# sipposip/pr-disagg-radar-gan

Hardware: AMD Instinct MI355X
Metric: cWGAN-GP train samples/sec, 24x16x16 tiles, bs=256 (higher is better)
Workload: dtype f32; 1 GPU; ndomain=16, 24h, bs=256 fp32, 1 critic step + 1 gen step (BASELINE configs[1]); batch_per_gpu=256, global_batch=256, n_critic=1, parallelism=dp1, world=1, rccl_ranks_seen=1, weights=random init (RandomNormal 0.02 / glorot_uniform), dropout 0.25 active

## Files before the change

pr_disagg_radar_gan_amd/csrc/rdgan_api.hip:

```cpp
#include <hip/hip_runtime.h>
#include <stdio.h>
#include <string.h>
#include <math.h>
#include <string>
#include <vector>
#include <algorithm>
#include <unordered_set>

#include "../../include/rdgan.h"
#include "rdgan_plan.h"
#include "rdgan_hostplan.h"
#include "rdgan_rng.h"
#include "rdgan_gemm.hip.h"
#include "rdgan_gemm_ws.hip.h"
#include "rdgan_gemm_ws16.hip.h"
#include "rdgan_gemm_f16.hip.h"
#include "rdgan_upconv16.hip.h"
#include "rdgan_upconv16b.hip.h"
#include "rdgan_upconv16t.hip.h"
#include "rdgan_elem.hip.h"
#include "rdgan_data.hip.h"
#include "rdgan_edge.hip.h"
#include "rdgan_d2slab16.hip.h"
#include "rdgan_d2fwd16.hip.h"
// ... 79 lines not shown
  float* dw6_part;
  int side_on = 1;
  int split3 = 0;
  int dense_slices = 0;
  uint64_t gver_in = 0, cver_in = 0;
  const float* gcache_ptr = nullptr; uint64_t gcache_ver = 0; int gcache_cfg = -1;
  const float* ccache_ptr = nullptr; uint64_t ccache_ver = 0; int ccache_cfg = -1;
  long form_builds[2] = {0, 0};
  int keep_gates = 0;
  void* gate_keep[5] = {nullptr, nullptr, nullptr, nullptr, nullptr};
  int gate_keep_B = 0;
  hipStream_t side = nullptr;
  hipEvent_t ev_fork = nullptr, ev_join = nullptr, ev_cw = nullptr, ev_g[4] = {nullptr, nullptr, nullptr, nullptr};
  int* d_flag;
  int fwd_ahead = -1;
  hipStream_t ahead = nullptr;
  hipEvent_t ev_ahead_fork = nullptr, ev_ahead_done = nullptr;
  float* kpartial_ahead = nullptr;
  int* flag_ahead = nullptr;
  bool ahead_pending = false;
  const float *ahead_gp = nullptr, *ahead_z = nullptr, *ahead_cond = nullptr;
  int ahead_B = 0;
  uint64_t ahead_gver = 0;
  std::unordered_set<const void*> lds_attr_done;
  int prof_launches = 0;
  std::vector<RdLaunchRec> launch_recs;
  size_t launch_used = 0;
  char cur_kernel[48] = {0};
  double flops_acc = 0;
  unsigned prof_mask = 0;
  std::vector<hipEvent_t> ev_start[RDGAN_NUM_TAGS], ev_stop[RDGAN_NUM_TAGS];
  size_t ev_used[RDGAN_NUM_TAGS] = {0};
};

#define RD_CHECK(h, call)                                                        \
  do {                                                                           \
    hipError_t e_ = (call);                                                      \
    if (e_ != hipSuccess) {                                                      \
      char b_[512];                                                              \
      snprintf(b_, sizeof b_, "%s:%d %s -> %s", __FILE__, __LINE__, #call, hipGetErrorString(e_)); \
      if (h) (h)->err = b_;                                                      \
      return (int)e_;                                                            \
    }                                                                            \
  } while (0)
#define RD_TRY(expr)            \
  do {                          \
// ... 689 lines not shown
    h->DWT[0] = h->DWT[1] = nullptr;
    for (int l = 2; l <= 4; ++l) carve(h->DWT[l], 27L * dch[l - 1] * dch[l]);
    carve(h->W1T, 64 * h->ldp1);
    carve(h->W1P, 27L * h->CP * 64); carve(h->dW1P, 27L * h->CP * 64);
    h->GWT[0] = nullptr;
    for (int l = 1; l <= 3; ++l) carve(h->GWT[l], 27L * gch[l - 1] * gch[l]);
    carve(h->W9T, 64 * 32);
    h->GWC[0] = h->GWD[0] = nullptr;
    for (int l = 1; l <= 3; ++l) { carve(h->GWC[l], 64L * gch[l - 1] * gch[l]); carve(h->GWD[l], 64L * gch[l - 1] * gch[l]); }
    carve(h->dWc, 64L * 256 * 256);
    {
      size_t ne = 0, ns = 0;
      for (int l = 1; l <= 3; ++l) {
        const int* sd = h->gdim[l - 1];
        ne = std::max(ne, (size_t)(sd[0] + 1) * sd[1] * sd[2] * gch[l - 1]);
        ns = std::max(ns, (size_t)sd[0] * 4 * sd[1] * sd[2] * gch[l]);
      }
      h->fE[0] = h->fU[0] = nullptr;
      for (int l = 1; l <= 3; ++l) {
        const int* sd = h->gdim[l - 1];
        carve(h->fE[l], MB * (size_t)(sd[0] + 1) * sd[1] * sd[2] * gch[l - 1]);
        carve(h->fU[l], 48L * gch[l - 1] * gch[l]);
      }
      carve(h->fdE, MB * ne); carve(h->fgS, MB * ns);
      {
        float* p = nullptr;
        h->bU[0] = nullptr;
        for (int l = 1; l <= 3; ++l) { carve(p, 24L * gch[l - 1] * gch[l] + 8); h->bU[l] = p; }
        carve(p, 24L * 256 * 256 + 8); h->bUT = p;
        const long KP128 = (h->n_in + 127) / 128 * 128;
        carve(p, (long)((MB + 31) / 32 * 32) * KP128 / 2 + 8); h->xcat16 = p;
        carve(p, (long)h->n_nodes * KP128 / 2 + 8); h->bW0 = p;
        h->bWF[0] = h->bWF[1] = h->bWB[0] = h->bWB[1] = nullptr;
        for (int l = 2; l <= 4; ++l) {
          carve(p, 27L * dch[l - 1] * dch[l] / 2 + 8); h->bWF[l] = p;
          carve(p, 27L * dch[l - 1] * dch[l] / 2 + 8); h->bWB[l] = p;
        }
        h->bG1F[0] = nullptr;
        for (int l = 1; l <= 3; ++l) { carve(p, 32L * gch[l - 1] * gch[l] + 8); h->bG1F[l] = p; }
        carve(p, 32L * 256 * 256 + 8); h->bG1B = p;
        h->fWF[0] = h->fWF[1] = h->fWB[0] = h->fWB[1] = h->fG1F[0] = nullptr;
        for (int l = 2; l <= 4; ++l) {
          carve(p, 27L * dch[l - 1] * dch[l] / 2 + 8); h->fWF[l] = p;
          carve(p, 27L * dch[l - 1] * dch[l] / 2 + 8); h->fWB[l] = p;
        }
        for (int l = 1; l <= 3; ++l) { carve(p, 32L * gch[l - 1] * gch[l] + 8); h->fG1F[l] = p; }
        carve(p, 32L * 256 * 256 + 8); h->fG1B = p;
// ... 8 lines not shown
      }
      carve(h->fdU, 48L * 256 * 256); carve(h->fUT, 48L * 256 * 256);
    }
    { float* f = nullptr; carve(f, 64); if (pass == 1) { h->d_flag = (int*)f; h->flag_ahead = (int*)f + 32; } }
    carve(h->g9b_tmp, 64);
    carve(h->ubias_part, 32 * 8 * 64);
    carve(h->gp_part, (size_t)MB * 64);
    carve(h->dw6_part, (size_t)16 * h->F);
    if (pass == 0) {
      h->ws_bytes = off + 256;
      e = hipMalloc((void**)&h->ws, h->ws_bytes);
      if (e != hipSuccess) { (void)hipFree(h->d_plans); delete h; return (int)e; }
      (void)hipMemset(h->ws, 0, h->ws_bytes);
    }
  }
  {
    bool ok = hipStreamCreateWithFlags(&h->side, hipStreamNonBlocking) == hipSuccess;
    hipEvent_t* evs[] = {&h->ev_fork, &h->ev_join, &h->ev_cw, &h->ev_g[1], &h->ev_g[2], &h->ev_g[3]};
    for (hipEvent_t* e2 : evs) ok = ok && hipEventCreateWithFlags(e2, hipEventDisableTiming) == hipSuccess;
    if (!ok) { h->side_on = 0; (void)hipGetLastError(); }
    bool ok2 = hipStreamCreateWithFlags(&h->ahead, hipStreamNonBlocking) == hipSuccess;
    ok2 = ok2 && hipEventCreateWithFlags(&h->ev_ahead_fork, hipEventDisableTiming) == hipSuccess;
    ok2 = ok2 && hipEventCreateWithFlags(&h->ev_ahead_done, hipEventDisableTiming) == hipSuccess;
    if (!ok2) { h->ahead = nullptr; (void)hipGetLastError(); }
  }
  *out = h;
  return 0;
}

extern "C" void rdgan_destroy(rdgan_handle* h) {
  if (!h) return;
  if (h->side) { (void)hipStreamSynchronize(h->side); (void)hipStreamDestroy(h->side); }
  if (h->ahead) { (void)hipStreamSynchronize(h->ahead); (void)hipStreamDestroy(h->ahead); }
  for (hipEvent_t e2 : {h->ev_fork, h->ev_join, h->ev_cw, h->ev_g[1], h->ev_g[2], h->ev_g[3], h->ev_ahead_fork, h->ev_ahead_done})
    if (e2) (void)hipEventDestroy(e2);
  for (auto& r : h->launch_recs) { (void)hipEventDestroy(r.e0); (void)hipEventDestroy(r.e1); }
  for (int t = 0; t < RDGAN_NUM_TAGS; ++t) {
    for (auto e : h->ev_start[t]) (void)hipEventDestroy(e);
    for (auto e : h->ev_stop[t]) (void)hipEventDestroy(e);
  }
  for (void* g : h->gate_keep) if (g) (void)hipFree(g);
  if (h->ws) (void)hipFree(h->ws);
  if (h->d_plans) (void)hipFree(h->d_plans);
  if (h->d_tab) (void)hipFree(h->d_tab);
  delete h;
}

extern "C" const char* rdgan_last_error(const rdgan_handle* h) { return h ? h->err.c_str() : "null handle"; }
extern "C" long rdgan_gen_param_count(const rdgan_handle* h) { return h ? h->n_gen : -1; }
extern "C" long rdgan_critic_param_count(const rdgan_handle* h) { return h ? h->n_critic : -1; }
extern "C" long rdgan_workspace_bytes(const rdgan_handle* h) { return h ? (long)h->ws_bytes : -1; }
extern "C" int rdgan_gen_param_layout(const rdgan_handle* h, long* offsets, long* sizes) {
  if (!h) return -2;
  for (int i = 0; i < 10; ++i) { if (offsets) offsets[i] = h->goff[i]; if (sizes) sizes[i] = h->gsz[i]; }
  return 10;
}
extern "C" int rdgan_critic_param_layout(const rdgan_handle* h, long* offsets, long* sizes) {
// ... 26 lines not shown
  if (!strcmp(name, "d2_wgrad_slab")) { h->d2_wgrad_slab = value ? 1 : 0; return 0; }
  if (!strcmp(name, "upwgrad_slab")) { h->upwgrad_slab = value ? 1 : 0; return 0; }
  if (!strcmp(name, "d1_dgrad_fused")) { h->d1_dgrad_fused = value ? 1 : 0; return 0; }
  if (!strcmp(name, "d1_wgrad16")) { h->d1_wgrad16 = value ? 1 : 0; return 0; }
  if (!strcmp(name, "wgrad_wide")) { h->wgrad_wide = value ? 1 : 0; return 0; }
  if (!strcmp(name, "conv_f16")) {
    if (value < 0 || value > 2) return bad_arg(h, "conv_f16: 0, 1 or 2 (2: regardless of the launch size)");
    h->conv_f16 = value; h->ccache_ver = 0; h->gcache_ver = 0; return 0;
  }
  if (!strcmp(name, "d2_fwd_slab")) { h->d2_fwd_slab = value ? 1 : 0; h->ccache_ver = 0; return 0; }
  if (!strcmp(name, "d2_gate_bits")) { h->d2_gate_bits = value ? 1 : 0; return 0; }
  if (!strcmp(name, "d2_slab")) { h->d2_slab = value ? 1 : 0; h->ccache_ver = 0; return 0; }
  if (!strcmp(name, "dense_wgrad_slices")) { h->dense_slices = value; return 0; }
  if (!strcmp(name, "keep_gates")) {
    h->keep_gates = value ? 1 : 0;
    h->gate_keep_B = 0;
    for (int l = 1; l <= 4 && h->keep_gates; ++l)
      if (!h->gate_keep[l]) RD_CHECK(h, hipMalloc(&h->gate_keep[l], (size_t)h->MB * h->dL[l] * h->dch[l] * sizeof(float)));
    return 0;
  }
  if (!strcmp(name, "split3")) { h->split3 = value ? 1 : 0; return 0; }
  if (!strcmp(name, "side_stream")) { h->side_on = (value && h->side) ? 1 : 0; return 0; }
  if (!strcmp(name, "gen_fwd_ahead")) { h->fwd_ahead = value < 0 ? -1 : (value ? 1 : 0); return 0; }
  if (!strcmp(name, "edge_kernels")) { h->edge_kernels = value < 0 ? 0 : (value > 2 ? 2 : value); return 0; }
  if (!strcmp(name, "sample_offset")) { if (value < 0) return bad_arg(h, "set_option: sample_offset < 0"); h->sample_offset = value; return 0; }
  if (!strcmp(name, "ws_ksplit")) { h->ws_ksplit = value < 0 ? 0 : (value > 8 ? 8 : value); return 0; }
  return bad_arg(h, "set_option: unknown option");
}

extern "C" int rdgan_set_weight_versions(rdgan_handle* h, uint64_t gen_version, uint64_t critic_version) {
  if (!h) return -2;
  h->gver_in = gen_version; h->cver_in = critic_version;
  return 0;
}
extern "C" int rdgan_form_builds(const rdgan_handle* h, long* gen_builds, long* critic_builds) {
  if (!h) return -2;
  if (gen_builds) *gen_builds = h->form_builds[0];
  if (critic_builds) *critic_builds = h->form_builds[1];
  return 0;
}

extern "C" int rdgan_profile(rdgan_handle* h, unsigned tag_mask) {
  if (!h) return -2;
  h->prof_mask = tag_mask;
  for (int t = 0; t < RDGAN_NUM_TAGS; ++t) {
    h->ev_used[t] = 0;
// ... 433 lines not shown
    e.gw = nd; e.ghw = nd * nd; e.gq = gq;
    if (a16) RD_TRY(launch_conv_a16(h, h->plans[PL_G9F], h->d_plans + PL_G9F, B, h->h3, h->W9T, 32, h->P9, e, st, -1, true, false));
    else
    RD_TRY(launch_conv(h, h->plans[PL_G9F], h->d_plans + PL_G9F, B, h->h3, h->W9T, 32, h->P9, e, st, -1));
    ProfScope ps(h, RDGAN_TAG_ELEMENTWISE, st);
    if (gq == 3) hipLaunchKernelGGL((k_tapsum_softmax<RDGAN_NHOURS, 3>), dim3((unsigned)((ncol + 63) / 64)), dim3(256), 0, st, h->P9,
                                    gp + h->goff[9], out, B, nd, nd, h->d_flag);
    else hipLaunchKernelGGL((k_tapsum_softmax<RDGAN_NHOURS, 9>), dim3((unsigned)((ncol + 63) / 64)), dim3(256), 0, st, h->P9,
                            gp + h->goff[9], out, B, nd, nd, h->d_flag);
  } else {
    if (a16) RD_TRY(launch_conv_a16(h, h->plans[PL_G9F], h->d_plans + PL_G9F, B, h->h3, h->W9T, 32, h->P9, epi_make(RD_EPI_PLAIN), st, -1,
                                    true, false));
    else
    RD_TRY(launch_conv(h, h->plans[PL_G9F], h->d_plans + PL_G9F, B, h->h3, h->W9T, 32, h->P9, epi_make(RD_EPI_PLAIN), st, -1));
    ProfScope ps(h, RDGAN_TAG_ELEMENTWISE, st);
    hipLaunchKernelGGL(k_colgather_softmax, dim3((unsigned)((ncol + 63) / 64)), dim3(64), 0, st, h->P9, gp + h->goff[9],
                       out, B, RDGAN_NHOURS, nd, nd, h->d_flag);
  }
  RD_CHECK(h, hipGetLastError());
  return 0;
}

static bool fwd_ahead_on(const rdgan_handle* h) { return h->ahead && h->ev_ahead_done && (h->fwd_ahead < 0 ? !h->a16 : h->fwd_ahead); }

static int ahead_drain(rdgan_handle* h, hipStream_t st) {
  if (!h->ahead_pending) return 0;
  h->ahead_pending = false;
  RD_CHECK(h, hipStreamWaitEvent(st, h->ev_ahead_done, 0));
  return 0;
}

static int ahead_issue(rdgan_handle* h, const float* gp, const float* z, const float* cond, int B, hipStream_t st) {
  RD_CHECK(h, hipEventRecord(h->ev_ahead_fork, st));
  RD_CHECK(h, hipStreamWaitEvent(h->ahead, h->ev_ahead_fork, 0));
  std::swap(h->kpartial, h->kpartial_ahead);
  std::swap(h->d_flag, h->flag_ahead);
  const int rc = gen_forward_impl(h, gp, z, cond, h->fake, B, h->ahead, h->ahead);
  std::swap(h->kpartial, h->kpartial_ahead);
  std::swap(h->d_flag, h->flag_ahead);
  RD_TRY(rc);
  RD_CHECK(h, hipEventRecord(h->ev_ahead_done, h->ahead));
  h->ahead_pending = true;
  h->ahead_gp = gp; h->ahead_z = z; h->ahead_cond = cond; h->ahead_B = B; h->ahead_gver = h->gver_in;
  return 0;
}

// ... 457 lines not shown
  h->ahead_pending = false;
  h->gate_keep_B = 0;
  if (!h->collapse)
    for (int l = 1; l <= 3; ++l)
      RD_TRY(launch_transpose(h, gp + h->goff[2 * l], h->GWT[l], 27, h->gch[l - 1], h->gch[l], h->gch[l - 1], st));
  hipStream_t ws = side_fork(h, st);
  if (!ahead) RD_TRY(gen_forward_impl(h, gp, z, cond, h->fake, B, st, ws));
  if (critic_ready_event) RD_CHECK(h, hipStreamWaitEvent(ws, (hipEvent_t)critic_ready_event, 0));
  RD_TRY(prep_critic_weights(h, dp, ws));
  RD_TRY(side_join(h, st, h->ev_cw));
  if (ahead) {
    RD_CHECK(h, hipStreamWaitEvent(st, h->ev_ahead_done, 0));
    std::swap(h->d_flag, h->flag_ahead);
  }
  {
    ProfScope ps(h, RDGAN_TAG_ELEMENTWISE, st);
    launch_build_critic_input(h, nullptr, h->fake, cond, B, 1, 0u, 0u, st);
  }
  RD_TRY(critic_forward_impl(h, dp, B, seed, st));
  RD_TRY(critic_dgrad_chain(h, dp, B, B, 1, seed, st));
  RD_TRY(critic_input_grad(h, dp, h->du[1], B, st));
  const bool a16 = h->a16 != 0;
  const long npix3 = (long)B * h->gpix[3];
  {
    ProfScope ps(h, RDGAN_TAG_ELEMENTWISE, st);
    long ncol = (long)B * nd * nd;
    hipLaunchKernelGGL(k_softmax_bwd, dim3((unsigned)((ncol + 63) / 64)), dim3(64), 0, st, h->fake, h->g0, h->dl, B,
                       RDGAN_NHOURS, nd, nd);
  }
  const size_t g9_lds = 4 * (size_t)(nd + 2) * (nd + 2) * sizeof(float);
  const bool g9_direct = h->g9_direct && g9_lds <= 96 * 1024 &&
                         (size_t)B * (RDGAN_NHOURS / 2) * 1728 <= h->wpartial_cap;
  if (a16 && !g9_direct) return bad_arg(h, "bf16 storage mode needs the direct backward of the last conv (g9_direct)");
  if (g9_direct) {
    ProfScope ps(h, RDGAN_TAG_GCONV_WGRAD, st);
    const size_t lds = std::max<size_t>(g9_lds, 4 * 27 * 16 * sizeof(f32x4));
    RD_TRY(ensure_lds(h, a16 ? (const void*)k_g9_bwd_pairs<rd_bf16_t> : (const void*)k_g9_bwd_pairs<float>, 96 * 1024));
    int nwg;
    if (h->edge_kernels && g9w_mfma_ok(nd, npix3) && (size_t)std::min<long>((npix3 + 127) / 128, 768) * 1728 <= h->wpartial_cap) {
      const size_t lds_m = g9w_mfma_lds(a16);
      RD_TRY(ensure_lds(h, a16 ? (const void*)k_g9_wgrad_mfma<rd_bf16_t> : (const void*)k_g9_wgrad_mfma<float>, lds_m));
      nwg = (int)std::min<long>((npix3 + 127) / 128, 768);
      LaunchScope ls(h, PL_G9B, RD_KIND_WGRAD, B, 2.0 * npix3 * 64 * 27, st);
      RD_KNAME(h, "k_g9_wgrad_mfma<%s>", a16 ? "bf16" : "f32");
      h->flops_acc += 2.0 * npix3 * 64 * 27;
      if (a16) hipLaunchKernelGGL(k_g9_wgrad_mfma<rd_bf16_t>, dim3(nwg), dim3(256), lds_m, st, h->dl, (const rd_bf16_t*)h->h3, h->wpartial,
                                  npix3, RDGAN_NHOURS, nd, nd, ilog2(nd));
      else hipLaunchKernelGGL(k_g9_wgrad_mfma<float>, dim3(nwg), dim3(256), lds_m, st, h->dl, (const float*)h->h3, h->wpartial,
                              npix3, RDGAN_NHOURS, nd, nd, ilog2(nd));
    } else {
      RD_TRY(ensure_lds(h, a16 ? (const void*)k_g9_wgrad_pairs<rd_bf16_t> : (const void*)k_g9_wgrad_pairs<float>, 96 * 1024));
      const int nunits = B * (RDGAN_NHOURS / 2);
      nwg = std::min(nunits, 3072);
      if (a16) hipLaunchKernelGGL(k_g9_wgrad_pairs<rd_bf16_t>, dim3(nwg), dim3(256), lds, st, h->dl, (const rd_bf16_t*)h->h3, h->wpartial,
                                  RDGAN_NHOURS, nd, nd, nunits);
      else hipLaunchKernelGGL(k_g9_wgrad_pairs<float>, dim3(nwg), dim3(256), lds, st, h->dl, (const float*)h->h3, h->wpartial,
                              RDGAN_NHOURS, nd, nd, nunits);
    }
    hipLaunchKernelGGL(k_reduce_partials, dim3((1728 + 15) / 16), dim3(rd_reduce_threads(nwg)), 0, st, h->wpartial, nwg, 1728, grad + h->goff[8]);
  } else {
    {
      ProfScope ps(h, RDGAN_TAG_ELEMENTWISE, st);
      hipLaunchKernelGGL(k_dl_im2col, dim3(ew_blocks(npix3 * 8)), dim3(256), 0, st, h->dl, h->P9, B, RDGAN_NHOURS, nd, nd);
    }
    RD_TRY(launch_wgrad(h, h->plans[PL_G9B], h->d_plans + PL_G9B, B, h->P9, h->h3, grad + h->goff[8], h->wpartial,
                        h->wpartial_cap, st, RDGAN_TAG_GCONV_WGRAD));
    RD_TRY(launch_conv(h, h->plans[PL_G9B], h->d_plans + PL_G9B, B, h->P9, gp + h->goff[8], 64, h->gh3,
                       epi_make(RD_EPI_PLAIN), st, RDGAN_TAG_GCONV_DGRAD));
  }
  {
    hipStream_t cs = side_fork(h, st);
    RD_TRY(launch_colsum(h, h->dl, npix3 / 64, 64, h->g9b_tmp, cs));
    RD_TRY(launch_colsum(h, h->g9b_tmp, 64, 1, grad + h->goff[9], cs));
  }
  float* hs[4] = {h->h0, h->h1, h->h2, h->h3};
  float* rs[4] = {nullptr, h->r1, h->r2, h->r3};
  float* dys[4] = {nullptr, h->dy1, h->dy2, h->gh3};
  float* gups[4] = {nullptr, h->gup1, h->gup2, h->gup3};
  const int col = h->collapse;
  if (col) {
    RdSliceMap map;
    collapsed_dgrad_slice_map(map.src);
    for (int l = 1; l <= 3; ++l) {
      if (gen_block_fast(h, l, fast_bwd_on(h))) continue;
      if (gen_block_fast(h, l, fast_fwd_on(h)))
        hipLaunchKernelGGL(k_collapse_weights, dim3(ew_blocks(16L * h->gch[l - 1] * h->gch[l])), dim3(256), 0, st,
                           gp + h->goff[2 * l], h->GWC[l], h->gch[l - 1] * h->gch[l]);
      if (a16) continue;
      hipLaunchKernelGGL(k_transpose_map, dim3((h->gch[l] + 31) / 32, (h->gch[l - 1] + 31) / 32, 64), dim3(256), 0, st,
                         h->GWC[l], h->GWD[l], h->gch[l - 1], h->gch[l], map);
    }
  }
  for (int l = 3; l >= 1; --l) {
    const bool fast = gen_block_fast(h, l, fast_bwd_on(h));
    if (l == 3 && g9_direct) {
      ProfScope ps(h, RDGAN_TAG_ELEMENTWISE, st);
      if (a16 && !fast && h->g9_bwd_mfma && (nd * nd) % 32 == 0) {
        const int PP = nd <= 16 ? 4 : 1;
        const size_t lds9 = (size_t)(2 * PP + 2) * (nd + 2) * (nd + 2) * sizeof(float);
        const int nunits = B * (RDGAN_NHOURS / 2 / PP);
        RD_TRY(ensure_lds(h, (const void*)k_g9_bwd_mfma16, lds9));
        hipLaunchKernelGGL(k_g9_bwd_mfma16, dim3((unsigned)std::min(nunits, PP > 1 ? 768 : 1536)), dim3(256), lds9, st, h->dl, gp + h->goff[8],
                           (const rd_bf16_t*)hs[3], rs[3], (rd_bf16_t*)dys[3], nunits, RDGAN_NHOURS, nd, nd, PP);
      } else
      if (a16) hipLaunchKernelGGL(k_g9_bwd_pairs<rd_bf16_t>, dim3(B * (RDGAN_NHOURS / 2)), dim3(256), g9_lds, st, h->dl, gp + h->goff[8],
                                  (const rd_bf16_t*)hs[3], rs[3], (rd_bf16_t*)dys[3], fast ? (rd_bf16_t*)h->fgS : (rd_bf16_t*)nullptr,
                                  RDGAN_NHOURS, nd, nd);
      else hipLaunchKernelGGL(k_g9_bwd_pairs<float>, dim3(B * (RDGAN_NHOURS / 2)), dim3(256), g9_lds, st, h->dl, gp + h->goff[8],
                              (const float*)hs[3], rs[3], dys[3], fast ? h->fgS : (float*)nullptr, RDGAN_NHOURS, nd, nd);
      RD_CHECK(h, hipGetLastError());
    } else if (fast) {
      ProfScope ps(h, RDGAN_TAG_ELEMENTWISE, st);
      const long HW = (long)h->gdim[l][1] * h->gdim[l][2];
      RD_TRY(launch_pn_bwd_pairs(h, l == 3 ? h->gh3 : gups[l + 1], hs[l], rs[l], dys[l], h->fgS, (long)B * h->gdim[l - 1][0] * HW,
                                 HW, h->gch[l], st, a16));
    } else {
      ProfScope ps(h, RDGAN_TAG_ELEMENTWISE, st);
      if (l == 3) RD_TRY(launch_pn_bwd(h, h->gh3, hs[3], rs[3], dys[3], npix3, 64, 0, 0, 0, 0, st, a16));
      else RD_TRY(launch_pn_bwd(h, gups[l + 1], hs[l], rs[l], dys[l], (long)B * h->gpix[l], h->gch[l], col ? 0 : 1,
                                h->gdim[l][0], h->gdim[l][1], h->gdim[l][2], st, a16));
    }
    const long cc = (long)h->gch[l - 1] * h->gch[l];
    if (fast) {
      const int* sd = h->gdim[l - 1];
      const int D = sd[0];
      const long P = (long)sd[1] * sd[2] * h->gch[l - 1];
      RdWeightMap wm;
      fastd_weight_map(wm);
      {
        ProfScope ps(h, RDGAN_TAG_ELEMENTWISE, st);
        if (!gen_block_fast(h, l, fast_fwd_on(h))) {
          const dim3 dg(ew_blocks((long)B * (D + 1) * P / 4));
          if (a16) hipLaunchKernelGGL(k_diff_d<rd_bf16_t>, dg, dim3(256), 0, st, (const rd_bf16_t*)hs[l - 1], (rd_bf16_t*)h->fE[l], B, D, P);
          else
          hipLaunchKernelGGL(k_diff_d<float>, dg, dim3(256), 0, st, (const float*)hs[l - 1],
                             h->fE[l], B, D, P);
          hipLaunchKernelGGL(k_weight_transform, dim3(ew_blocks(48L * cc / 4)), dim3(256), 0, st, gp + h->goff[2 * l], h->fU[l],
                             (int)cc, 48, wm);
        }
      }
      const float* wsrc[3] = {h->fE[l], hs[l - 1], h->fE[l]};
      const float* wdy[3] = {dys[l], h->fgS, dys[l]};
      for (int g = 0; g < 3; ++g) {
        int pl = PL_F1WA + 3 * g + l - 1;
        if (!a16 && h->wgrad_boxes && h->border_boxes && h->wave_spec && wgrad_box_ok(h->plans[PL_F1WAX + 3 * g + l - 1]) &&
            (h->border_boxes >= 2 || plan_flops(h->plans[PL_F1WAX + 3 * g + l - 1], 1) < 0.8 * plan_flops(h->plans[pl], 1)))
          pl = PL_F1WAX + 3 * g + l - 1;
        if (a16) {
          if (!wgrad16_ok(h->plans[pl], B)) return bad_arg(h, "bf16 storage mode: no bf16 weight-gradient tile for this block");
          RD_TRY(launch_wgrad16(h, h->plans[pl], h->d_plans + pl, B, wsrc[g], wdy[g], h->fdU, h->wpartial, h->wpartial_cap, st,
                                RDGAN_TAG_GCONV_WGRAD));
        } else
        RD_TRY(launch_wgrad(h, h->plans[pl], h->d_plans + pl, B, wsrc[g], wdy[g], h->fdU, h->wpartial, h->wpartial_cap, st,
                            RDGAN_TAG_GCONV_WGRAD));
      }
      hipLaunchKernelGGL(k_weight_transform_adj, dim3(ew_blocks(27L * cc / 4)), dim3(256), 0, st, h->fdU, grad + h->goff[2 * l],
                         (int)cc, 48, wm);
      RD_TRY(launch_colsum(h, dys[l], (long)B * h->gpix[l], h->gch[l], grad + h->goff[2 * l + 1], side_fork(h, st), a16));
      const int pbs = PL_F1BS + l - 1, pbe = PL_F1BE + l - 1;
      RdEpi eb = epi_make(RD_EPI_PLAIN);
      eb.out16 = a16;
      if (a16) {
        RdSliceMap map;
        fastd_dgrad_slice_map(map.src);
        {
          ProfScope ps(h, RDGAN_TAG_ELEMENTWISE, st);
          hipLaunchKernelGGL(k_blocks_to_bf16, dim3((unsigned)std::min<long>((cc / 8 + 255) / 256, 64), 48), dim3(256), 0, st,
                             h->fU[l], (unsigned short*)h->bUT, cc, map);
        }
        RD_TRY(launch_conv16(h, h->plans[pbs], h->d_plans + pbs, B, h->fgS, h->bUT, gups[l], eb, st, RDGAN_TAG_GCONV_DGRAD));
        RD_TRY(launch_conv16(h, h->plans[pbe], h->d_plans + pbe, B, dys[l], h->bUT, h->fdE, eb, st, RDGAN_TAG_GCONV_DGRAD));
      } else {
        {
          RdSliceMap map;
          fastd_dgrad_slice_map(map.src);
          hipLaunchKernelGGL(k_transpose_map, dim3((h->gch[l] + 31) / 32, (h->gch[l - 1] + 31) / 32, 48), dim3(256), 0, st, h->fU[l],
                             h->fUT, h->gch[l - 1], h->gch[l], map);
        }
        RD_TRY(launch_conv(h, h->plans[pbs], h->d_plans + pbs, B, h->fgS, h->fUT, h->gch[l - 1], gups[l], eb, st,
                           RDGAN_TAG_GCONV_DGRAD));
        RD_TRY(launch_conv(h, h->plans[pbe], h->d_plans + pbe, B, dys[l], h->fUT, h->gch[l - 1], h->fdE, eb, st,
                           RDGAN_TAG_GCONV_DGRAD));
      }
      {
        ProfScope ps(h, RDGAN_TAG_ELEMENTWISE, st);
        const dim3 cg(ew_blocks((long)B * D * P / 4));
        if (a16) hipLaunchKernelGGL(k_combine_dx<rd_bf16_t>, cg, dim3(256), 0, st, (rd_bf16_t*)gups[l], (const rd_bf16_t*)h->fdE, B, D, P);
        else hipLaunchKernelGGL(k_combine_dx<float>, cg, dim3(256), 0, st, gups[l], (const float*)h->fdE, B, D, P);
      }
    } else if (col) {
      int plf = PL_G1FC + l - 1, plb = gen_box_plan(h, PL_G1BC + l - 1, PL_G1BCX + l - 1, B);
      const int plfx = PL_G1FCX + l - 1;
      const bool wbox = h->wgrad_boxes && h->border_boxes && h->wave_spec && wgrad_box_ok(h->plans[plfx]) &&
                        (h->border_boxes >= 2 || plan_flops(h->plans[plfx], 1) < 0.8 * plan_flops(h->plans[plf], 1));
      bool bias_done = false;
      if (a16 && l == 3 && h->upwgrad_slab && h->nd == 16) {
        ProfScope ps(h, RDGAN_TAG_GCONV_WGRAD, st);
        LaunchScope ls(h, plf, RD_KIND_WGRAD, B, plan_flops(h->plans[plf], B), st);
        RD_KNAME(h, "k_upconv_wgrad_slab16<bf16>");
        h->flops_acc += plan_flops(h->plans[plf], B);
        const int G = 6 * B >= 64 ? 32 : 8;
        if ((size_t)G * 64 * RD_UWG_TILE > h->wpartial_cap) return bad_arg(h, "upconv wgrad: partial workspace too small");
        RD_TRY(ensure_lds(h, (const void*)k_upconv_wgrad_slab16, RD_UWG_LDS));
        hipLaunchKernelGGL(k_upconv_wgrad_slab16, dim3(8 * G), dim3(512), RD_UWG_LDS, st, (const rd_bf16_t*)hs[l - 1],
                           (const rd_bf16_t*)dys[l], h->wpartial, B, G, h->ubias_part);
        hipLaunchKernelGGL(k_upconv_wgrad_fold, dim3(64 * RD_UWG_TILE / 4 / 256), dim3(256), 0, st, h->wpartial, G, h->dWc);
        hipLaunchKernelGGL(k_reduce_partials, dim3(64 / 16), dim3(rd_reduce_threads(8 * G)), 0, st, h->ubias_part, 8 * G, 64, grad + h->goff[2 * l + 1]);
        bias_done = true;
        RD_CHECK(h, hipGetLastError());
      } else if (a16 && l == 2 && h->upwgrad_slab && h->nd == 16) {
        ProfScope ps(h, RDGAN_TAG_GCONV_WGRAD, st);
        LaunchScope ls(h, plf, RD_KIND_WGRAD, B, plan_flops(h->plans[plf], B), st);
        RD_KNAME(h, "k_upconv2_wgrad_slab16<bf16>");
        h->flops_acc += plan_flops(h->plans[plf], B);
        const int G = 8;
        if ((size_t)G * 64 * RD_UW2_TILE > h->wpartial_cap) return bad_arg(h, "upconv wgrad: partial workspace too small");
        RD_TRY(ensure_lds(h, (const void*)k_upconv2_wgrad_slab16, RD_UW2_LDS));
        hipLaunchKernelGGL(k_upconv2_wgrad_slab16, dim3(32 * G), dim3(512), RD_UW2_LDS, st, (const rd_bf16_t*)hs[l - 1],
                           (const rd_bf16_t*)dys[l], h->wpartial, B, G, h->ubias_part);
        hipLaunchKernelGGL(k_upconv2_wgrad_fold, dim3(64 * RD_UW2_TILE / 4 / 256), dim3(256), 0, st, h->wpartial, G, h->dWc);
        hipLaunchKernelGGL(k_reduce_partials, dim3(128 / 16), dim3(rd_reduce_threads(8 * G)), 0, st, h->ubias_part, 8 * G, 128, grad + h->goff[2 * l + 1]);
        bias_done = true;
        RD_CHECK(h, hipGetLastError());
      } else if (a16) {
        if (wbox && wgrad16_ok(h->plans[plfx], B)) plf = plfx;
        if (!wgrad16_ok(h->plans[plf], B)) return bad_arg(h, "bf16 storage mode: no bf16 weight-gradient tile for this block");
        RD_TRY(launch_wgrad16(h, h->plans[plf], h->d_plans + plf, B, hs[l - 1], dys[l], h->dWc, h->wpartial, h->wpartial_cap, st,
                              RDGAN_TAG_GCONV_WGRAD));
      } else {
      if (wbox) plf = plfx;
      RD_TRY(launch_wgrad(h, h->plans[plf], h->d_plans + plf, B, hs[l - 1], dys[l], h->dWc, h->wpartial, h->wpartial_cap,
                          st, RDGAN_TAG_GCONV_WGRAD));
      }
      hipLaunchKernelGGL(k_fold_collapsed_wgrad, dim3(ew_blocks(27L * cc / 4)), dim3(256), 0, st, h->dWc,
                         grad + h->goff[2 * l], (int)cc);
      if (!bias_done)
      RD_TRY(launch_colsum(h, dys[l], (long)B * h->gpix[l], h->gch[l], grad + h->goff[2 * l + 1], side_fork(h, st), a16));
      if (a16) {
        RdSliceMap map;
        collapsed_dgrad_slice_map(map.src);
        hipLaunchKernelGGL(k_blocks_to_bf16, dim3((unsigned)std::min<long>((cc / 8 + 255) / 256, 64), 64), dim3(256), 0, st,
                           h->GWC[l], (unsigned short*)h->bG1B, cc, map, h->conv_f16 ? (unsigned short*)h->fG1B : nullptr, h->gch[l]);
        RdEpi eb = epi_make(RD_EPI_PLAIN);
        eb.out16 = 1;
        RD_TRY(launch_conv16(h, h->plans[plb], h->d_plans + plb, B, dys[l], h->bG1B, gups[l], eb, st, RDGAN_TAG_GCONV_DGRAD,
                             h->conv_f16 ? h->fG1B : nullptr));
      } else
      RD_TRY(launch_conv(h, h->plans[plb], h->d_plans + plb, B, dys[l], h->GWD[l], h->gch[l - 1], gups[l],
                         epi_make(RD_EPI_PLAIN), st, RDGAN_TAG_GCONV_DGRAD));
    } else {
      int plf = PL_G1F + l - 1, plb = PL_G1B + l - 1;
      RD_TRY(launch_wgrad(h, h->plans[plf], h->d_plans + plf, B, hs[l - 1], dys[l], grad + h->goff[2 * l], h->wpartial,
                          h->wpartial_cap, st, RDGAN_TAG_GCONV_WGRAD));
      RD_TRY(launch_colsum(h, dys[l], (long)B * h->gpix[l], h->gch[l], grad + h->goff[2 * l + 1], side_fork(h, st)));
      RD_TRY(launch_conv(h, h->plans[plb], h->d_plans + plb, B, dys[l], h->GWT[l], h->gch[l - 1], gups[l],
                         epi_make(RD_EPI_PLAIN), st, RDGAN_TAG_GCONV_DGRAD));
    }
  }
  {
    ProfScope ps(h, RDGAN_TAG_ELEMENTWISE, st);
    const dim3 lg(ew_blocks((long)B * h->gpix[0] * 64));
    if (col && a16)
      hipLaunchKernelGGL(k_lrelu_bwd<rd_bf16_t>, lg, dim3(256), 0, st, (const rd_bf16_t*)h->gup1, (const rd_bf16_t*)h->h0, h->ga0,
                         (long)B * h->gpix[0] * 64);
    else if (col)
      hipLaunchKernelGGL(k_lrelu_bwd<float>, lg, dim3(256), 0, st, (const float*)h->gup1, (const float*)h->h0, h->ga0,
                         (long)B * h->gpix[0] * 64);
    else
      hipLaunchKernelGGL(k_pool_lrelu_bwd, lg, dim3(256), 0, st, h->gup1, h->h0,
                         h->ga0, (long)B * h->gpix[0], h->gdim[0][0], h->gdim[0][1], h->gdim[0][2], 256);
  }
  RD_TRY(launch_wgrad(h, h->plans[PL_GDENSE], h->d_plans + PL_GDENSE, B, h->xcat, h->ga0, grad + h->goff[0], h->wpartial,
                      h->wpartial_cap, st, RDGAN_TAG_GCONV_WGRAD));
  RD_TRY(launch_colsum(h, h->ga0, B, h->n_nodes, grad + h->goff[1], side_fork(h, st)));
  RD_TRY(side_join(h, st, h->ev_join));
  {
    ProfScope ps(h, RDGAN_TAG_ELEMENTWISE, st);
    hipLaunchKernelGGL(k_gen_loss, dim3(1), dim3(256), 0, st, h->v, grad + h->n_gen, B, h->d_flag);
  }
  RD_CHECK(h, hipGetLastError());
  return 0;
}

extern "C" int rdgan_adam(float* params, const float* grad, float* v, long n, int t, float lr, float beta2, float eps,
                          float grad_scale, void* stream) {
  if (!params || !grad || !v || n < 1 || t < 1) return -2;
  float lr_t = lr * sqrtf(1.0f - powf(beta2, (float)t));
  hipLaunchKernelGGL(k_adam, dim3(ew_blocks(n / 4 + 1)), dim3(256), 0, (hipStream_t)stream, params, grad, v, n, lr_t, beta2,
                     eps, grad_scale);
  return (int)hipGetLastError();
}

struct TmpPlan {
  RdPlan host; RdPlan* dev = nullptr; RdRow* tab = nullptr;
  int upload() {
    std::vector<RdRow> t;
    if (!plan_build_tables(host, t)) return -2;
    hipError_t e = hipMalloc((void**)&tab, sizeof(RdRow) * t.size());
// ... 776 lines not shown
```

Before: 23580 samples/s.

## Fork generator weight-gradient kernels onto a second stream to overlap data-gradient chain

Generator backward weight-gradient launches (last conv, fast-path blocks, upconv blocks, dense layer) move onto the 'ahead' stream, forked by events from the main stream. The data-gradient convs stay on the main stream, so the two chains can run concurrently. A second fgS scratch buffer, used by block 2, plus per-buffer events stop the overlapping blocks from overwriting a shared buffer, and a join event merges the streams before the loss kernel. It is on by default only in fp32 mode (not a16). It costs extra events, workspace and possible contention for compute units between the streams.

```diff
diff --git a/pr_disagg_radar_gan_amd/csrc/rdgan_api.hip b/pr_disagg_radar_gan_amd/csrc/rdgan_api.hip
--- a/pr_disagg_radar_gan_amd/csrc/rdgan_api.hip
+++ b/pr_disagg_radar_gan_amd/csrc/rdgan_api.hip
@@ -125,6 +125,9 @@
   const float *ahead_gp = nullptr, *ahead_z = nullptr, *ahead_cond = nullptr;
   int ahead_B = 0;
   uint64_t ahead_gver = 0;
+  int wgrad_fork = -1;
+  hipEvent_t ev_wg_fork = nullptr, ev_wg_join = nullptr, ev_fgs[2] = {nullptr, nullptr};
+  float* fgS2 = nullptr;
   std::unordered_set<const void*> lds_attr_done;
   int prof_launches = 0;
   std::vector<RdLaunchRec> launch_recs;
@@ -860,7 +863,7 @@
         carve(h->fE[l], MB * (size_t)(sd[0] + 1) * sd[1] * sd[2] * gch[l - 1]);
         carve(h->fU[l], 48L * gch[l - 1] * gch[l]);
       }
-      carve(h->fdE, MB * ne); carve(h->fgS, MB * ns);
+      carve(h->fdE, MB * ne); carve(h->fgS, MB * ns); carve(h->fgS2, MB * ns);
       {
         float* p = nullptr;
         h->bU[0] = nullptr;
@@ -915,6 +918,8 @@
     bool ok2 = hipStreamCreateWithFlags(&h->ahead, hipStreamNonBlocking) == hipSuccess;
     ok2 = ok2 && hipEventCreateWithFlags(&h->ev_ahead_fork, hipEventDisableTiming) == hipSuccess;
     ok2 = ok2 && hipEventCreateWithFlags(&h->ev_ahead_done, hipEventDisableTiming) == hipSuccess;
+    for (hipEvent_t* e2 : {&h->ev_wg_fork, &h->ev_wg_join, &h->ev_fgs[0], &h->ev_fgs[1]})
+      ok2 = ok2 && hipEventCreateWithFlags(e2, hipEventDisableTiming) == hipSuccess;
     if (!ok2) { h->ahead = nullptr; (void)hipGetLastError(); }
   }
   *out = h;
@@ -925,7 +930,8 @@
   if (!h) return;
   if (h->side) { (void)hipStreamSynchronize(h->side); (void)hipStreamDestroy(h->side); }
   if (h->ahead) { (void)hipStreamSynchronize(h->ahead); (void)hipStreamDestroy(h->ahead); }
-  for (hipEvent_t e2 : {h->ev_fork, h->ev_join, h->ev_cw, h->ev_g[1], h->ev_g[2], h->ev_g[3], h->ev_ahead_fork, h->ev_ahead_done})
+  for (hipEvent_t e2 : {h->ev_fork, h->ev_join, h->ev_cw, h->ev_g[1], h->ev_g[2], h->ev_g[3], h->ev_ahead_fork, h->ev_ahead_done,
+                        h->ev_wg_fork, h->ev_wg_join, h->ev_fgs[0], h->ev_fgs[1]})
     if (e2) (void)hipEventDestroy(e2);
   for (auto& r : h->launch_recs) { (void)hipEventDestroy(r.e0); (void)hipEventDestroy(r.e1); }
   for (int t = 0; t < RDGAN_NUM_TAGS; ++t) {
@@ -998,6 +1004,7 @@
   if (!strcmp(name, "split3")) { h->split3 = value ? 1 : 0; return 0; }
   if (!strcmp(name, "side_stream")) { h->side_on = (value && h->side) ? 1 : 0; return 0; }
   if (!strcmp(name, "gen_fwd_ahead")) { h->fwd_ahead = value < 0 ? -1 : (value ? 1 : 0); return 0; }
+  if (!strcmp(name, "gen_wgrad_fork")) { h->wgrad_fork = value < 0 ? -1 : (value ? 1 : 0); return 0; }
   if (!strcmp(name, "edge_kernels")) { h->edge_kernels = value < 0 ? 0 : (value > 2 ? 2 : value); return 0; }
   if (!strcmp(name, "sample_offset")) { if (value < 0) return bad_arg(h, "set_option: sample_offset < 0"); h->sample_offset = value; return 0; }
   if (!strcmp(name, "ws_ksplit")) { h->ws_ksplit = value < 0 ? 0 : (value > 8 ? 8 : value); return 0; }
@@ -1477,6 +1484,9 @@
 }
 
 static bool fwd_ahead_on(const rdgan_handle* h) { return h->ahead && h->ev_ahead_done && (h->fwd_ahead < 0 ? !h->a16 : h->fwd_ahead); }
+static bool wgrad_fork_on(const rdgan_handle* h) {
+  return h->ahead && h->ev_wg_fork && h->ev_wg_join && h->ev_fgs[1] && (h->wgrad_fork < 0 ? !h->a16 : h->wgrad_fork);
+}
 
 static int ahead_drain(rdgan_handle* h, hipStream_t st) {
   if (!h->ahead_pending) return 0;
@@ -1980,6 +1990,15 @@
   RD_TRY(critic_input_grad(h, dp, h->du[1], B, st));
   const bool a16 = h->a16 != 0;
   const long npix3 = (long)B * h->gpix[3];
+  const bool wfork = wgrad_fork_on(h);
+  hipStream_t wb = st;
+  auto wgrad_branch = [&]() -> int {
+    if (!wfork) return 0;
+    RD_CHECK(h, hipEventRecord(h->ev_wg_fork, st));
+    RD_CHECK(h, hipStreamWaitEvent(h->ahead, h->ev_wg_fork, 0));
+    wb = h->ahead;
+    return 0;
+  };
   {
     ProfScope ps(h, RDGAN_TAG_ELEMENTWISE, st);
     long ncol = (long)B * nd * nd;
@@ -1991,7 +2010,8 @@
                          (size_t)B * (RDGAN_NHOURS / 2) * 1728 <= h->wpartial_cap;
   if (a16 && !g9_direct) return bad_arg(h, "bf16 storage mode needs the direct backward of the last conv (g9_direct)");
   if (g9_direct) {
-    ProfScope ps(h, RDGAN_TAG_GCONV_WGRAD, st);
+    RD_TRY(wgrad_branch());
+    ProfScope ps(h, RDGAN_TAG_GCONV_WGRAD, wb);
     const size_t lds = std::max<size_t>(g9_lds, 4 * 27 * 16 * sizeof(f32x4));
     RD_TRY(ensure_lds(h, a16 ? (const void*)k_g9_bwd_pairs<rd_bf16_t> : (const void*)k_g9_bwd_pairs<float>, 96 * 1024));
     int nwg;
@@ -1999,30 +2019,31 @@
       const size_t lds_m = g9w_mfma_lds(a16);
       RD_TRY(ensure_lds(h, a16 ? (const void*)k_g9_wgrad_mfma<rd_bf16_t> : (const void*)k_g9_wgrad_mfma<float>, lds_m));
       nwg = (int)std::min<long>((npix3 + 127) / 128, 768);
-      LaunchScope ls(h, PL_G9B, RD_KIND_WGRAD, B, 2.0 * npix3 * 64 * 27, st);
+      LaunchScope ls(h, PL_G9B, RD_KIND_WGRAD, B, 2.0 * npix3 * 64 * 27, wb);
       RD_KNAME(h, "k_g9_wgrad_mfma<%s>", a16 ? "bf16" : "f32");
       h->flops_acc += 2.0 * npix3 * 64 * 27;
-      if (a16) hipLaunchKernelGGL(k_g9_wgrad_mfma<rd_bf16_t>, dim3(nwg), dim3(256), lds_m, st, h->dl, (const rd_bf16_t*)h->h3, h->wpartial,
+      if (a16) hipLaunchKernelGGL(k_g9_wgrad_mfma<rd_bf16_t>, dim3(nwg), dim3(256), lds_m, wb, h->dl, (const rd_bf16_t*)h->h3, h->wpartial,
                                   npix3, RDGAN_NHOURS, nd, nd, ilog2(nd));
-      else hipLaunchKernelGGL(k_g9_wgrad_mfma<float>, dim3(nwg), dim3(256), lds_m, st, h->dl, (const float*)h->h3, h->wpartial,
+      else hipLaunchKernelGGL(k_g9_wgrad_mfma<float>, dim3(nwg), dim3(256), lds_m, wb, h->dl, (const float*)h->h3, h->wpartial,
                               npix3, RDGAN_NHOURS, nd, nd, ilog2(nd));
     } else {
       RD_TRY(ensure_lds(h, a16 ? (const void*)k_g9_wgrad_pairs<rd_bf16_t> : (const void*)k_g9_wgrad_pairs<float>, 96 * 1024));
       const int nunits = B * (RDGAN_NHOURS / 2);
       nwg = std::min(nunits, 3072);
-      if (a16) hipLaunchKernelGGL(k_g9_wgrad_pairs<rd_bf16_t>, dim3(nwg), dim3(256), lds, st, h->dl, (const rd_bf16_t*)h->h3, h->wpartial,
+      if (a16) hipLaunchKernelGGL(k_g9_wgrad_pairs<rd_bf16_t>, dim3(nwg), dim3(256), lds, wb, h->dl, (const rd_bf16_t*)h->h3, h->wpartial,
                                   RDGAN_NHOURS, nd, nd, nunits);
-      else hipLaunchKernelGGL(k_g9_wgrad_pairs<float>, dim3(nwg), dim3(256), lds, st, h->dl, (const float*)h->h3, h->wpartial,
+      else hipLaunchKernelGGL(k_g9_wgrad_pairs<float>, dim3(nwg), dim3(256), lds, wb, h->dl, (const float*)h->h3, h->wpartial,
                               RDGAN_NHOURS, nd, nd, nunits);
     }
-    hipLaunchKernelGGL(k_reduce_partials, dim3((1728 + 15) / 16), dim3(rd_reduce_threads(nwg)), 0, st, h->wpartial, nwg, 1728, grad + h->goff[8]);
+    hipLaunchKernelGGL(k_reduce_partials, dim3((1728 + 15) / 16), dim3(rd_reduce_threads(nwg)), 0, wb, h->wpartial, nwg, 1728, grad + h->goff[8]);
   } else {
     {
       ProfScope ps(h, RDGAN_TAG_ELEMENTWISE, st);
       hipLaunchKernelGGL(k_dl_im2col, dim3(ew_blocks(npix3 * 8)), dim3(256), 0, st, h->dl, h->P9, B, RDGAN_NHOURS, nd, nd);
     }
+    RD_TRY(wgrad_branch());
     RD_TRY(launch_wgrad(h, h->plans[PL_G9B], h->d_plans + PL_G9B, B, h->P9, h->h3, grad + h->goff[8], h->wpartial,
-                        h->wpartial_cap, st, RDGAN_TAG_GCONV_WGRAD));
+                        h->wpartial_cap, wb, RDGAN_TAG_GCONV_WGRAD));
     RD_TRY(launch_conv(h, h->plans[PL_G9B], h->d_plans + PL_G9B, B, h->P9, gp + h->goff[8], 64, h->gh3,
                        epi_make(RD_EPI_PLAIN), st, RDGAN_TAG_GCONV_DGRAD));
   }
@@ -2049,8 +2070,12 @@
                          h->GWC[l], h->GWD[l], h->gch[l - 1], h->gch[l], map);
     }
   }
+  bool fgs_branch[2] = {false, false};
   for (int l = 3; l >= 1; --l) {
     const bool fast = gen_block_fast(h, l, fast_bwd_on(h));
+    const int fgi = wfork && l == 2 ? 1 : 0;
+    float* const fgs = fgi ? h->fgS2 : h->fgS;
+    if (fast && fgs_branch[fgi]) RD_CHECK(h, hipStreamWaitEvent(st, h->ev_fgs[fgi], 0));
     if (l == 3 && g9_direct) {
       ProfScope ps(h, RDGAN_TAG_ELEMENTWISE, st);
       if (a16 && !fast && h->g9_bwd_mfma && (nd * nd) % 32 == 0) {
@@ -2062,15 +2087,15 @@
                            (const rd_bf16_t*)hs[3], rs[3], (rd_bf16_t*)dys[3], nunits, RDGAN_NHOURS, nd, nd, PP);
       } else
       if (a16) hipLaunchKernelGGL(k_g9_bwd_pairs<rd_bf16_t>, dim3(B * (RDGAN_NHOURS / 2)), dim3(256), g9_lds, st, h->dl, gp + h->goff[8],
-                                  (const rd_bf16_t*)hs[3], rs[3], (rd_bf16_t*)dys[3], fast ? (rd_bf16_t*)h->fgS : (rd_bf16_t*)nullptr,
+                                  (const rd_bf16_t*)hs[3], rs[3], (rd_bf16_t*)dys[3], fast ? (rd_bf16_t*)fgs : (rd_bf16_t*)nullptr,
                                   RDGAN_NHOURS, nd, nd);
       else hipLaunchKernelGGL(k_g9_bwd_pairs<float>, dim3(B * (RDGAN_NHOURS / 2)), dim3(256), g9_lds, st, h->dl, gp + h->goff[8],
-                              (const float*)hs[3], rs[3], dys[3], fast ? h->fgS : (float*)nullptr, RDGAN_NHOURS, nd, nd);
+                              (const float*)hs[3], rs[3], dys[3], fast ? fgs : (float*)nullptr, RDGAN_NHOURS, nd, nd);
       RD_CHECK(h, hipGetLastError());
     } else if (fast) {
       ProfScope ps(h, RDGAN_TAG_ELEMENTWISE, st);
       const long HW = (long)h->gdim[l][1] * h->gdim[l][2];
-      RD_TRY(launch_pn_bwd_pairs(h, l == 3 ? h->gh3 : gups[l + 1], hs[l], rs[l], dys[l], h->fgS, (long)B * h->gdim[l - 1][0] * HW,
+      RD_TRY(launch_pn_bwd_pairs(h, l == 3 ? h->gh3 : gups[l + 1], hs[l], rs[l], dys[l], fgs, (long)B * h->gdim[l - 1][0] * HW,
                                  HW, h->gch[l], st, a16));
     } else {
       ProfScope ps(h, RDGAN_TAG_ELEMENTWISE, st);
@@ -2098,7 +2123,8 @@
         }
       }
       const float* wsrc[3] = {h->fE[l], hs[l - 1], h->fE[l]};
-      const float* wdy[3] = {dys[l], h->fgS, dys[l]};
+      const float* wdy[3] = {dys[l], fgs, dys[l]};
+      RD_TRY(wgrad_branch());
       for (int g = 0; g < 3; ++g) {
         int pl = PL_F1WA + 3 * g + l - 1;
         if (!a16 && h->wgrad_boxes && h->border_boxes && h->wave_spec && wgrad_box_ok(h->plans[PL_F1WAX + 3 * g + l - 1]) &&
@@ -2106,13 +2132,14 @@
           pl = PL_F1WAX + 3 * g + l - 1;
         if (a16) {
           if (!wgrad16_ok(h->plans[pl], B)) return bad_arg(h, "bf16 storage mode: no bf16 weight-gradient tile for this block");
-          RD_TRY(launch_wgrad16(h, h->plans[pl], h->d_plans + pl, B, wsrc[g], wdy[g], h->fdU, h->wpartial, h->wpartial_cap, st,
+          RD_TRY(launch_wgrad16(h, h->plans[pl], h->d_plans + pl, B, wsrc[g], wdy[g], h->fdU, h->wpartial, h->wpartial_cap, wb,
                                 RDGAN_TAG_GCONV_WGRAD));
         } else
-        RD_TRY(launch_wgrad(h, h->plans[pl], h->d_plans + pl, B, wsrc[g], wdy[g], h->fdU, h->wpartial, h->wpartial_cap, st,
+        RD_TRY(launch_wgrad(h, h->plans[pl], h->d_plans + pl, B, wsrc[g], wdy[g], h->fdU, h->wpartial, h->wpartial_cap, wb,
                             RDGAN_TAG_GCONV_WGRAD));
       }
-      hipLaunchKernelGGL(k_weight_transform_adj, dim3(ew_blocks(27L * cc / 4)), dim3(256), 0, st, h->fdU, grad + h->goff[2 * l],
+      if (wfork) { RD_CHECK(h, hipEventRecord(h->ev_fgs[fgi], wb)); fgs_branch[fgi] = true; }
+      hipLaunchKernelGGL(k_weight_transform_adj, dim3(ew_blocks(27L * cc / 4)), dim3(256), 0, wb, h->fdU, grad + h->goff[2 * l],
                          (int)cc, 48, wm);
       RD_TRY(launch_colsum(h, dys[l], (long)B * h->gpix[l], h->gch[l], grad + h->goff[2 * l + 1], side_fork(h, st), a16));
       const int pbs = PL_F1BS + l - 1, pbe = PL_F1BE + l - 1;
@@ -2126,7 +2153,7 @@
           hipLaunchKernelGGL(k_blocks_to_bf16, dim3((unsigned)std::min<long>((cc / 8 + 255) / 256, 64), 48), dim3(256), 0, st,
                              h->fU[l], (unsigned short*)h->bUT, cc, map);
         }
-        RD_TRY(launch_conv16(h, h->plans[pbs], h->d_plans + pbs, B, h->fgS, h->bUT, gups[l], eb, st, RDGAN_TAG_GCONV_DGRAD));
+        RD_TRY(launch_conv16(h, h->plans[pbs], h->d_plans + pbs, B, fgs, h->bUT, gups[l], eb, st, RDGAN_TAG_GCONV_DGRAD));
         RD_TRY(launch_conv16(h, h->plans[pbe], h->d_plans + pbe, B, dys[l], h->bUT, h->fdE, eb, st, RDGAN_TAG_GCONV_DGRAD));
       } else {
         {
@@ -2135,7 +2162,7 @@
           hipLaunchKernelGGL(k_transpose_map, dim3((h->gch[l] + 31) / 32, (h->gch[l - 1] + 31) / 32, 48), dim3(256), 0, st, h->fU[l],
                              h->fUT, h->gch[l - 1], h->gch[l], map);
         }
-        RD_TRY(launch_conv(h, h->plans[pbs], h->d_plans + pbs, B, h->fgS, h->fUT, h->gch[l - 1], gups[l], eb, st,
+        RD_TRY(launch_conv(h, h->plans[pbs], h->d_plans + pbs, B, fgs, h->fUT, h->gch[l - 1], gups[l], eb, st,
                            RDGAN_TAG_GCONV_DGRAD));
         RD_TRY(launch_conv(h, h->plans[pbe], h->d_plans + pbe, B, dys[l], h->fUT, h->gch[l - 1], h->fdE, eb, st,
                            RDGAN_TAG_GCONV_DGRAD));
@@ -2152,45 +2179,46 @@
       const bool wbox = h->wgrad_boxes && h->border_boxes && h->wave_spec && wgrad_box_ok(h->plans[plfx]) &&
                         (h->border_boxes >= 2 || plan_flops(h->plans[plfx], 1) < 0.8 * plan_flops(h->plans[plf], 1));
       bool bias_done = false;
+      RD_TRY(wgrad_branch());
       if (a16 && l == 3 && h->upwgrad_slab && h->nd == 16) {
-        ProfScope ps(h, RDGAN_TAG_GCONV_WGRAD, st);
-        LaunchScope ls(h, plf, RD_KIND_WGRAD, B, plan_flops(h->plans[plf], B), st);
+        ProfScope ps(h, RDGAN_TAG_GCONV_WGRAD, wb);
+        LaunchScope ls(h, plf, RD_KIND_WGRAD, B, plan_flops(h->plans[plf], B), wb);
         RD_KNAME(h, "k_upconv_wgrad_slab16<bf16>");
         h->flops_acc += plan_flops(h->plans[plf], B);
         const int G = 6 * B >= 64 ? 32 : 8;
         if ((size_t)G * 64 * RD_UWG_TILE > h->wpartial_cap) return bad_arg(h, "upconv wgrad: partial workspace too small");
         RD_TRY(ensure_lds(h, (const void*)k_upconv_wgrad_slab16, RD_UWG_LDS));
-        hipLaunchKernelGGL(k_upconv_wgrad_slab16, dim3(8 * G), dim3(512), RD_UWG_LDS, st, (const rd_bf16_t*)hs[l - 1],
+        hipLaunchKernelGGL(k_upconv_wgrad_slab16, dim3(8 * G), dim3(512), RD_UWG_LDS, wb, (const rd_bf16_t*)hs[l - 1],
                            (const rd_bf16_t*)dys[l], h->wpartial, B, G, h->ubias_part);
-        hipLaunchKernelGGL(k_upconv_wgrad_fold, dim3(64 * RD_UWG_TILE / 4 / 256), dim3(256), 0, st, h->wpartial, G, h->dWc);
-        hipLaunchKernelGGL(k_reduce_partials, dim3(64 / 16), dim3(rd_reduce_threads(8 * G)), 0, st, h->ubias_part, 8 * G, 64, grad + h->goff[2 * l + 1]);
+        hipLaunchKernelGGL(k_upconv_wgrad_fold, dim3(64 * RD_UWG_TILE / 4 / 256), dim3(256), 0, wb, h->wpartial, G, h->dWc);
+        hipLaunchKernelGGL(k_reduce_partials, dim3(64 / 16), dim3(rd_reduce_threads(8 * G)), 0, wb, h->ubias_part, 8 * G, 64, grad + h->goff[2 * l + 1]);
         bias_done = true;
         RD_CHECK(h, hipGetLastError());
       } else if (a16 && l == 2 && h->upwgrad_slab && h->nd == 16) {
-        ProfScope ps(h, RDGAN_TAG_GCONV_WGRAD, st);
-        LaunchScope ls(h, plf, RD_KIND_WGRAD, B, plan_flops(h->plans[plf], B), st);
+        ProfScope ps(h, RDGAN_TAG_GCONV_WGRAD, wb);
+        LaunchScope ls(h, plf, RD_KIND_WGRAD, B, plan_flops(h->plans[plf], B), wb);
         RD_KNAME(h, "k_upconv2_wgrad_slab16<bf16>");
         h->flops_acc += plan_flops(h->plans[plf], B);
         const int G = 8;
         if ((size_t)G * 64 * RD_UW2_TILE > h->wpartial_cap) return bad_arg(h, "upconv wgrad: partial workspace too small");
         RD_TRY(ensure_lds(h, (const void*)k_upconv2_wgrad_slab16, RD_UW2_LDS));
-        hipLaunchKernelGGL(k_upconv2_wgrad_slab16, dim3(32 * G), dim3(512), RD_UW2_LDS, st, (const rd_bf16_t*)hs[l - 1],
+        hipLaunchKernelGGL(k_upconv2_wgrad_slab16, dim3(32 * G), dim3(512), RD_UW2_LDS, wb, (const rd_bf16_t*)hs[l - 1],
                            (const rd_bf16_t*)dys[l], h->wpartial, B, G, h->ubias_part);
-        hipLaunchKernelGGL(k_upconv2_wgrad_fold, dim3(64 * RD_UW2_TILE / 4 / 256), dim3(256), 0, st, h->wpartial, G, h->dWc);
-        hipLaunchKernelGGL(k_reduce_partials, dim3(128 / 16), dim3(rd_reduce_threads(8 * G)), 0, st, h->ubias_part, 8 * G, 128, grad + h->goff[2 * l + 1]);
+        hipLaunchKernelGGL(k_upconv2_wgrad_fold, dim3(64 * RD_UW2_TILE / 4 / 256), dim3(256), 0, wb, h->wpartial, G, h->dWc);
+        hipLaunchKernelGGL(k_reduce_partials, dim3(128 / 16), dim3(rd_reduce_threads(8 * G)), 0, wb, h->ubias_part, 8 * G, 128, grad + h->goff[2 * l + 1]);
         bias_done = true;
         RD_CHECK(h, hipGetLastError());
       } else if (a16) {
         if (wbox && wgrad16_ok(h->plans[plfx], B)) plf = plfx;
         if (!wgrad16_ok(h->plans[plf], B)) return bad_arg(h, "bf16 storage mode: no bf16 weight-gradient tile for this block");
-        RD_TRY(launch_wgrad16(h, h->plans[plf], h->d_plans + plf, B, hs[l - 1], dys[l], h->dWc, h->wpartial, h->wpartial_cap, st,
+        RD_TRY(launch_wgrad16(h, h->plans[plf], h->d_plans + plf, B, hs[l - 1], dys[l], h->dWc, h->wpartial, h->wpartial_cap, wb,
                               RDGAN_TAG_GCONV_WGRAD));
       } else {
       if (wbox) plf = plfx;
       RD_TRY(launch_wgrad(h, h->plans[plf], h->d_plans + plf, B, hs[l - 1], dys[l], h->dWc, h->wpartial, h->wpartial_cap,
-                          st, RDGAN_TAG_GCONV_WGRAD));
+                          wb, RDGAN_TAG_GCONV_WGRAD));
       }
-      hipLaunchKernelGGL(k_fold_collapsed_wgrad, dim3(ew_blocks(27L * cc / 4)), dim3(256), 0, st, h->dWc,
+      hipLaunchKernelGGL(k_fold_collapsed_wgrad, dim3(ew_blocks(27L * cc / 4)), dim3(256), 0, wb, h->dWc,
                          grad + h->goff[2 * l], (int)cc);
       if (!bias_done)
       RD_TRY(launch_colsum(h, dys[l], (long)B * h->gpix[l], h->gch[l], grad + h->goff[2 * l + 1], side_fork(h, st), a16));
@@ -2208,8 +2236,9 @@
                          epi_make(RD_EPI_PLAIN), st, RDGAN_TAG_GCONV_DGRAD));
     } else {
       int plf = PL_G1F + l - 1, plb = PL_G1B + l - 1;
+      RD_TRY(wgrad_branch());
       RD_TRY(launch_wgrad(h, h->plans[plf], h->d_plans + plf, B, hs[l - 1], dys[l], grad + h->goff[2 * l], h->wpartial,
-                          h->wpartial_cap, st, RDGAN_TAG_GCONV_WGRAD));
+                          h->wpartial_cap, wb, RDGAN_TAG_GCONV_WGRAD));
       RD_TRY(launch_colsum(h, dys[l], (long)B * h->gpix[l], h->gch[l], grad + h->goff[2 * l + 1], side_fork(h, st)));
       RD_TRY(launch_conv(h, h->plans[plb], h->d_plans + plb, B, dys[l], h->GWT[l], h->gch[l - 1], gups[l],
                          epi_make(RD_EPI_PLAIN), st, RDGAN_TAG_GCONV_DGRAD));
@@ -2228,10 +2257,15 @@
       hipLaunchKernelGGL(k_pool_lrelu_bwd, lg, dim3(256), 0, st, h->gup1, h->h0,
                          h->ga0, (long)B * h->gpix[0], h->gdim[0][0], h->gdim[0][1], h->gdim[0][2], 256);
   }
+  RD_TRY(wgrad_branch());
   RD_TRY(launch_wgrad(h, h->plans[PL_GDENSE], h->d_plans + PL_GDENSE, B, h->xcat, h->ga0, grad + h->goff[0], h->wpartial,
-                      h->wpartial_cap, st, RDGAN_TAG_GCONV_WGRAD));
+                      h->wpartial_cap, wb, RDGAN_TAG_GCONV_WGRAD));
   RD_TRY(launch_colsum(h, h->ga0, B, h->n_nodes, grad + h->goff[1], side_fork(h, st)));
   RD_TRY(side_join(h, st, h->ev_join));
+  if (wb != st) {
+    RD_CHECK(h, hipEventRecord(h->ev_wg_join, wb));
+    RD_CHECK(h, hipStreamWaitEvent(st, h->ev_wg_join, 0));
+  }
   {
     ProfScope ps(h, RDGAN_TAG_ELEMENTWISE, st);
     hipLaunchKernelGGL(k_gen_loss, dim3(1), dim3(256), 0, st, h->v, grad + h->n_gen, B, h->d_flag);
```

Measured after the change: 23880 samples/s, median of 6. 1.01x the previous value.
